# HybridRobotics/ilqr-iterative-tasks

Hardware: AMD Instinct MI355X
Metric: batched iLQR iterations/s (n=6,m=2,N=20) (higher is better)
Workload: dtype f64

## Files before the change

### ilqr_iterative_tasks_amd/csrc/i2lqr_abi.hip

```cpp
#include <hip/hip_runtime.h>
#include <dlfcn.h>
#include <rccl/rccl.h>

#include <atomic>
#include <cmath>
#include <cstdarg>
#include <cstdio>
#include <cstdlib>
#include <cstring>
#include <mutex>
#include <new>
#include <unordered_set>

#include "../../include/i2lqr.h"
#include "i2lqr_devcfg.hpp"
#include "i2lqr_geometry.hpp"
#include "i2lqr_group.h"
#include "i2lqr_lane.hpp"
#include "i2lqr_select.hpp"
#include "i2lqr_wave.hpp"

#include "i2lqr_lane12.h"

#define I2LQR_DRY_RUN_LANE 1
// ... 173 lines not shown
int debug_check(int rc, void* stream) {
#ifdef I2LQR_DEBUG
  if (rc != I2LQR_OK) return rc;
  unsigned long long* w = i2lqr::debug_trap_word();
  if (!w) return rc;
  hipStreamCaptureStatus cap = hipStreamCaptureStatusNone;
  if (hipStreamIsCapturing((hipStream_t)stream, &cap) == hipSuccess &&
      cap != hipStreamCaptureStatusNone)
    return rc;
  if (hipStreamSynchronize((hipStream_t)stream) != hipSuccess)
    return fail(I2LQR_ERR_LAUNCH, "debug build: the stream reported an error");
  unsigned long long rec = 0;
  if (hipMemcpy(&rec, w, sizeof(rec), hipMemcpyDeviceToHost) != hipSuccess)
    return fail(I2LQR_ERR_LAUNCH, "debug build: could not read the violation record");
  if (rec) {
    (void)hipMemset(w, 0, sizeof(rec));
    static const char* const names[] = {"?", "wave-kernel LDS slice", "eight-lane LDS slice",
                                        "sixteen-lane LDS slice", "quad12 HBM workspace slot",
                                        "lane kernel row of X", "lane kernel row of U / k",
                                        "lane kernel row of K", "lane kernel LDS word",
                                        "compaction row / problem index"};
    const int tag = (int)((rec >> 56) & 0x7f);
    return fail(I2LQR_ERR_LAUNCH, "debug build: index check failed: %s, index %lld, limit %lld",
                names[tag < 10 ? tag : 0], (long long)((rec >> 28) & 0xfffffff),
                (long long)(rec & 0xfffffff));
  }
#else
  (void)stream;
#endif
  return rc;
}
}

struct i2lqr_handle {
  i2lqr_config cfg;
  int lanes;
  size_t lds_bytes;
  int device;
  void* ws;
  int64_t ws_bytes;
  int64_t compact_min_batch;
  int opt_defer, opt_reroll, opt_lds_steps, opt_merge, opt_ckpt, opt_stagger;
  int wave_tail;
  int opt_pair;
  int opt_two_x;
  int opt_chunk_step;
  int opt_fuse;
  int opt_final_round;
  int opt_first_chunk;
  int opt_fstep;
  int opt_group;
  int opt_spec;
  int opt_group_ws;
  struct Epilogue {
    const int32_t* qfun;
    int outer_iter, max_relax_iter;
    void* cost_it;
    void* part;
    int64_t* best_idx;
    void* best_cost;
    bool fused;
  };
  static constexpr unsigned kTickets = 16;
  unsigned* ticket;
  std::atomic<unsigned> ticket_next;
  hipEvent_t ev_ready, ev_side_done;
  bool side_pending;
  DeviceGeometry geo;
};

namespace {
thread_local i2lqr_handle::Epilogue* t_epi = nullptr;
}

namespace {

enum FusedKernel { K_WAVE, K_GROUP, K_GROUP16, K_GROUP_WS, K_SPEC, K_SPEC16, K_QUAD, K_INVALID };
constexpr int64_t kAutoGroupBatch = 1024;
constexpr int64_t kAutoSpecBatch = 12288;

FusedKernel select_fused(const i2lqr_handle* h, int64_t B, bool early_exit, const char** why) {
  static const char* none = "";
  if (!why) why = &none;
  const bool m2 = h->cfg.m == 2 && h->cfg.n + h->cfg.m <= 8;
  const bool q16 = h->cfg.n + h->cfg.m == 16;
  if (m2) {
    const bool can = group_supported(h->cfg);
    if (h->opt_group == 8 && !can) {
      *why = "\"group_lanes\" = 8 needs a bicycle plant with Q = R = 0 and a horizon whose eight "
             "problem slices fit a CU's LDS";
      return K_INVALID;
    }
    const bool can_spec16 = group_spec_supported(h->cfg, 16), can_spec8 = group_spec_supported(h->cfg, 8);
    const bool spec16 = h->opt_group == 16 || (h->opt_group < 0 && can_spec16);
    const bool can_spec = spec16 ? can_spec16 : can_spec8;
    if (h->opt_spec == 1 && !can_spec) {
      *why = "\"speculate\" = 1 needs the eight- / sixteen-lane kernel and a horizon whose speculative "
             "buffers fit a CU's LDS";
      return K_INVALID;
    }
    if (can_spec && h->opt_group != 64 &&
        (h->opt_spec == 1 ||
         (h->opt_spec < 0 && h->opt_group < 0 && early_exit && B <= h->geo.scaled(kAutoSpecBatch))))
      return spec16 ? K_SPEC16 : K_SPEC;
    const bool can16 = group16_supported(h->cfg);
    if (h->opt_group == 16 && !can16) {
// ... 84 lines not shown
    IterArgs<T> a;
    a.B = B;
    a.n_iters = n_iters;
    a.early_exit = early_exit;
    a.X = (T*)X;
    a.U = (T*)U;
    a.x_term = (const T*)x_term;
    a.lamb = (T*)lamb;
    a.obs = (const T*)obs;
    a.cost = (T*)cost;
    a.K = (T*)K;
    a.k = (T*)k;
    a.iters = iters;
    a.status = status;
    a.dbg = nullptr;
    a.count = nullptr; a.count_max = 0; a.max_total = 0; a.set_stride = 0;
#ifdef I2LQR_STAMPS
    a.dbg = (unsigned long long*)h->ws;
#endif
    const char* why = "";
    const FusedKernel fk = select_fused(h, B, early_exit != 0, &why);
    if (t_epi && (fk == K_GROUP || fk == K_GROUP16 || fk == K_GROUP_WS)) {
      a.qfun = t_epi->qfun;
      a.outer_iter = t_epi->outer_iter;
      a.max_relax_iter = t_epi->max_relax_iter;
      a.cost_it = (T*)t_epi->cost_it;
      if (t_epi->best_idx) {
        a.pick_part = (MinPair<T>*)t_epi->part;
        a.pick_ticket = h->ticket + h->ticket_next.fetch_add(1, std::memory_order_relaxed) %
                                        i2lqr_handle::kTickets;
        a.best_idx = t_epi->best_idx;
        a.best_cost = (T*)t_epi->best_cost;
      }
      t_epi->fused = true;
    }
    switch (fk) {
      case K_INVALID:
        return fail(I2LQR_ERR_UNSUPPORTED, "%s", why);
      case K_SPEC:
      case K_SPEC16:
        if constexpr (m == 2 && n + m <= 8) {
          HIP_TRY(group_spec_iterate<T>(h->cfg, a, s, fk == K_SPEC16 ? 16 : 8));
          return I2LQR_OK;
        }
        break;
      case K_GROUP:
        if constexpr (m == 2 && n + m <= 8) {
          HIP_TRY(group_iterate<T>(h->cfg, a, s));
          return I2LQR_OK;
        }
        break;
      case K_GROUP16:
        if constexpr (m == 2 && n + m <= 8) {
          HIP_TRY(group16_iterate<T>(h->cfg, a, s));
          return I2LQR_OK;
        }
        break;
      case K_GROUP_WS:
        if constexpr (m == 2 && n + m <= 8) {
          HIP_TRY(group_iterate_ws<T>(h->cfg, a, h->ws, s));
          return I2LQR_OK;
        }
        break;
      case K_QUAD:
        if constexpr (n + m == 16) {
          HIP_TRY(quad_iterate<T>(h->cfg, a, h->ws, s));
          return I2LQR_OK;
        }
        break;
      case K_WAVE:
        break;
    }
    const size_t lds_f = fstep_lds_bytes(h->cfg.N);
    const int64_t waves_per_cu = (grid(B) + h->geo.cus - 1) / h->geo.cus;
    const bool fstep = kHasFstep && lds_f <= h->geo.default_dyn_lds &&
                       (h->opt_fstep >= 0 ? h->opt_fstep != 0
                                          : waves_per_cu * lds_f <= h->geo.lds_per_cu - 10 * 1024);
    if constexpr (kHasFstep) {
      if (fstep) {
        if (c.flags)
          hipLaunchKernelGGL((k_iterate<T, Sys, LANES, true, true>), dim3(grid(B)), dim3(64), lds_f,
                             s, c, a);
        else
          hipLaunchKernelGGL((k_iterate<T, Sys, LANES, false, true>), dim3(grid(B)), dim3(64), lds_f,
                             s, c, a);
        HIP_TRY(hipGetLastError());
        return I2LQR_OK;
      }
    }
    if (c.flags)
      hipLaunchKernelGGL((k_iterate<T, Sys, LANES, true>), dim3(grid(B)), dim3(64), h->lds_bytes, s,
                         c, a);
    else
      hipLaunchKernelGGL((k_iterate<T, Sys, LANES, false>), dim3(grid(B)), dim3(64), h->lds_bytes,
                         s, c, a);
    HIP_TRY(hipGetLastError());
    return I2LQR_OK;
  }
  static int names_pair(i2lqr_handle*, int64_t, int) { return 0; }
  static int solve_chained(i2lqr_handle* h, int64_t L, int k, void* X, void* U, const void* x_term,
                           void* lamb, const void* obs, void* cost, void* K, void* kk, int32_t* iters,
                           int32_t* status, hipStream_t s) {
    if constexpr (m == 2 && n + m <= 8) {
      if (h->opt_spec == 0 || h->opt_group == 8 || h->opt_group == 64 ||
          !group_spec_chain_supported(h->cfg, L))
        return fail(I2LQR_ERR_UNSUPPORTED, "chains run on the sixteen-lane speculative kernel: a "
                    "bicycle plant with Q = R = 0, at most %lld chains, a horizon whose three-wavefront "
// ... 879 lines not shown
    case I2LQR_SYS_QUAD12: n = 12; m = 4; break;
    default: return fail(I2LQR_ERR_INVALID, "unknown system_id %d", cfg->system_id);
  }
  if (cfg->n != n || cfg->m != m)
    return fail(I2LQR_ERR_INVALID, "system %d has n=%d m=%d, config says n=%d m=%d", cfg->system_id,
                n, m, cfg->n, cfg->m);
  if (cfg->N < 1 || cfg->N > I2LQR_MAX_HORIZON)
    return fail(I2LQR_ERR_INVALID, "horizon %d outside [1, %d]", cfg->N, I2LQR_MAX_HORIZON);
  if (cfg->dtype != I2LQR_F64 && cfg->dtype != I2LQR_F32)
    return fail(I2LQR_ERR_INVALID, "unknown dtype %d", cfg->dtype);
  if (cfg->layout != I2LQR_LAYOUT_PROBLEM_MAJOR && cfg->layout != I2LQR_LAYOUT_BATCH_MINOR &&
      cfg->layout != I2LQR_LAYOUT_BATCH_TILED)
    return fail(I2LQR_ERR_INVALID, "unknown layout %d", cfg->layout);
  if (!(cfg->dt > 0) || !(cfg->lamb_factor > 1) || cfg->max_iter < 0)
    return fail(I2LQR_ERR_INVALID, "need dt > 0, lamb_factor > 1, max_iter >= 0");
  for (int a = 0; a < m; a++)
    if (!(cfg->u_max[a] > 0)) return fail(I2LQR_ERR_INVALID, "u_max[%d] must be > 0", a);
  if (cfg->layout != I2LQR_LAYOUT_PROBLEM_MAJOR) {
    for (int i = 0; i < n; i++)
      for (int j = 0; j < i; j++)
        if (cfg->Q[i * I2LQR_MAX_N + j] != cfg->Q[j * I2LQR_MAX_N + i] ||
            cfg->Qt[i * I2LQR_MAX_N + j] != cfg->Qt[j * I2LQR_MAX_N + i])
          return fail(I2LQR_ERR_UNSUPPORTED, "the batch-minor / batch-tiled layouts need "
                      "symmetric Q and Qterminal (use the problem-major layout otherwise)");
    for (int a = 0; a < m; a++)
      for (int b = 0; b < a; b++)
        if (cfg->R[a * I2LQR_MAX_M + b] != cfg->R[b * I2LQR_MAX_M + a])
          return fail(I2LQR_ERR_UNSUPPORTED, "the batch-minor / batch-tiled layouts need a "
                      "symmetric R (use the problem-major layout otherwise)");
  }
  int ndev = 0;
#ifdef I2LQR_DRY_RUN
  const bool dry_run = dry::on();
#else
  constexpr bool dry_run = false;
#endif
  if (!dry_run && (hipGetDeviceCount(&ndev) != hipSuccess || ndev <= 0))
    return fail(I2LQR_ERR_NODEVICE, "no HIP device visible (this library has no CPU path)");
  i2lqr_handle* h = new (std::nothrow) i2lqr_handle;
  if (!h) return fail(I2LQR_ERR_LAUNCH, "out of host memory");
  h->cfg = *cfg;
  h->geo = device_geometry();
  if (h->geo.wave != 64) {
    const int w = h->geo.wave;
    delete h;
    return fail(I2LQR_ERR_UNSUPPORTED, "the kernels are built for 64-lane wavefronts (gfx950), this "
                "device reports %d", w);
  }
  h->ws = nullptr;
  h->ws_bytes = 0;
  h->compact_min_batch = -1;
  h->opt_defer = h->opt_reroll = h->opt_lds_steps = h->opt_fstep = h->opt_group = -1;
  h->opt_merge = h->opt_ckpt = h->opt_spec = h->opt_stagger = h->opt_group_ws = -1;
  h->wave_tail = -1;
  h->opt_first_chunk = -1;
  h->opt_fuse = -1;
  h->opt_final_round = -1;
  h->opt_chunk_step = -1;
  h->opt_pair = -1;
  h->opt_two_x = -1;
  h->ticket = nullptr;
  h->ticket_next.store(0);
  h->ev_ready = h->ev_side_done = nullptr;
  h->side_pending = false;
  constexpr size_t kTicketBytes = i2lqr_handle::kTickets * sizeof(unsigned);
  if (dry_run) {
#ifdef I2LQR_DRY_RUN
    static unsigned fake_tickets[i2lqr_handle::kTickets];
    h->device = 0;
    h->ticket = fake_tickets;
    dry::allow(fake_tickets, sizeof(fake_tickets));
#endif
  } else if (hipGetDevice(&h->device) != hipSuccess ||
      hipMalloc((void**)&h->ticket, kTicketBytes) != hipSuccess ||
      hipMemset(h->ticket, 0, kTicketBytes) != hipSuccess) {
    if (h->ticket) (void)hipFree(h->ticket);
    delete h;
    return fail(I2LQR_ERR_LAUNCH, "could not set up the handle's device state: %s",
                hipGetErrorString(hipGetLastError()));
  }
  const int rc = prepare_dispatch(h);
  if (rc != I2LQR_OK) {
    (void)hipFree(h->ticket);
    delete h;
    return rc;
  }
  {
    std::lock_guard<std::mutex> lock(g_live_mu);
    live_handles().insert(h);
  }
  *out = h;
  g_err[0] = 0;
  return I2LQR_OK;
}

int64_t i2lqr_dry_run(int32_t op, void* p, int64_t n) {
#ifdef I2LQR_DRY_RUN
  switch (op) {
    case 0: return dry::on() ? 1 : 0;
    case 1: if (!dry::on()) break; dry::allow(p, (size_t)n); return 0;
    case 2: if (!dry::on()) break; dry::reset(); return 0;
    case 3: if (!dry::on()) break; return dry::report((char*)p, n);
    default: return fail(I2LQR_ERR_INVALID, "i2lqr_dry_run: unknown operation %d", op);
  }
  return fail(I2LQR_ERR_UNSUPPORTED, "dry-run launches need I2LQR_DRY_RUN=1 in the environment");
#else
// ... 94 lines not shown
  for (int a = 0; a < cfg->m; a++)
    for (int b = 0; b < cfg->m; b++) {
      if (cfg->R[a * I2LQR_MAX_M + b] != 0.0) weights = true;
      if (cfg->R[a * I2LQR_MAX_M + b] != cfg->R[b * I2LQR_MAX_M + a]) lane_ok = false;
    }
  int64_t from;
  switch (cfg->system_id) {
    case I2LQR_SYS_BICYCLE4:
    case I2LQR_SYS_BICYCLE6:
      from = weights ? kLaneFromWeights
                     : (early_exit ? lane_from(*cfg).solve : lane_from(*cfg).iterate);
      break;
    case I2LQR_SYS_QUAD12: {
      const LaneFrom q = kLaneFromQuad[cfg->N <= 31 ? 0 : 1][cfg->dtype == I2LQR_F64 ? 0 : 1];
      from = weights ? kLaneFromWeights : (early_exit ? q.solve : q.iterate);
      if (cfg->dtype != I2LQR_F64 && weights) lane_ok = false;
      break;
    }
    default: return fail(I2LQR_ERR_INVALID, "unknown system_id %d", cfg->system_id);
  }
  from = device_geometry().scaled_from(from);
  if (!lane_ok || B < from) return I2LQR_LAYOUT_PROBLEM_MAJOR;
  return B % 64 == 0 ? I2LQR_LAYOUT_BATCH_TILED : I2LQR_LAYOUT_BATCH_MINOR;
}

int i2lqr_set_compaction(i2lqr_handle* h, int64_t min_batch) {
  if (!h) return fail(I2LQR_ERR_INVALID, "null handle");
  if (h->cfg.layout == I2LQR_LAYOUT_PROBLEM_MAJOR && min_batch > 0)
    return fail(I2LQR_ERR_UNSUPPORTED, "compaction applies to the batch-minor / batch-tiled layouts");
  h->compact_min_batch = min_batch < 0 ? -1 : min_batch;
  return I2LQR_OK;
}

int i2lqr_set_option(i2lqr_handle* h, const char* name, int64_t value) {
  if (!h || !name) return fail(I2LQR_ERR_INVALID, "null handle or option name");
  if (value < -1 || value > 0x7fffffff) return fail(I2LQR_ERR_INVALID, "option value out of range");
  const int v = (int)value;
  if (!strcmp(name, "defer_states")) h->opt_defer = v < 0 ? -1 : (v != 0);
  else if (!strcmp(name, "reroll_nominal")) h->opt_reroll = v < 0 ? -1 : (v != 0);
  else if (!strcmp(name, "lds_gain_steps")) h->opt_lds_steps = v;
  else if (!strcmp(name, "merge_inputs")) h->opt_merge = v < 0 ? -1 : (v != 0);
  else if (!strcmp(name, "checkpoint_states")) h->opt_ckpt = v < 0 ? -1 : (v != 0);
  else if (!strcmp(name, "stagger")) h->opt_stagger = v;
  else if (!strcmp(name, "per_step_jacobians")) h->opt_fstep = v < 0 ? -1 : (v != 0);
  else if (!strcmp(name, "wave_tail")) h->wave_tail = v < 0 ? -1 : (v > 65536 ? 65536 : v);
  else if (!strcmp(name, "first_chunk")) h->opt_first_chunk = v < 1 ? -1 : (v > 1024 ? 1024 : v);
  else if (!strcmp(name, "helper_wavefront")) h->opt_pair = v < 0 ? -1 : (v != 0);
  else if (!strcmp(name, "state_buffers")) h->opt_two_x = v < 0 ? -1 : (v != 0);
  else if (!strcmp(name, "chunk_step")) h->opt_chunk_step = v < 1 ? -1 : (v > 1024 ? 1024 : v);
  else if (!strcmp(name, "fused_compaction")) h->opt_fuse = v < 0 ? -1 : (v != 0);
  else if (!strcmp(name, "final_round")) h->opt_final_round = v < 0 ? -1 : (v > 20 ? 20 : v);
  else if (!strcmp(name, "speculate")) h->opt_spec = v < 0 ? -1 : (v != 0);
  else if (!strcmp(name, "group_workspace")) h->opt_group_ws = v < 0 ? -1 : (v != 0);
  else if (!strcmp(name, "debug_self_test")) {
#ifdef I2LQR_DEBUG
    unsigned long long* w = i2lqr::debug_trap_word();
    double* buf = nullptr;
    HIP_TRY(hipMalloc((void**)&buf, 8 * sizeof(double)));
    hipLaunchKernelGGL(k_debug_self_test, dim3(1), dim3(64), 0, (hipStream_t)0, buf, w);
    const int rc = debug_check(I2LQR_OK, nullptr);
    (void)hipFree(buf);
    return rc;
#else
    return fail(I2LQR_ERR_UNSUPPORTED, "\"debug_self_test\" exists in the index-checked debug build "
                "only (make -C ilqr_iterative_tasks_amd/csrc debug)");
#endif
  }
  else if (!strcmp(name, "group_lanes")) {
    if (v != -1 && v != 8 && v != 16 && v != 64)
      return fail(I2LQR_ERR_INVALID, "\"group_lanes\" is 8, 16, 64 or -1");
    h->opt_group = v;
  }
  else return fail(I2LQR_ERR_INVALID, "unknown option '%s'", name);
  return I2LQR_OK;
}

static const char* kernel_name(const i2lqr_handle* h, int64_t B, bool early_exit) {
  if (!h) return "";
  if (h->cfg.layout != I2LQR_LAYOUT_PROBLEM_MAJOR) {
    if (h->cfg.system_id == I2LQR_SYS_QUAD12) return "k_lane_iterate_rows";
    return names_pair_dispatch(const_cast<i2lqr_handle*>(h), B, early_exit ? 1 : 0) == 1
               ? "k_lane_iterate_pair" : "k_lane_iterate";
  }
  switch (select_fused(h, B, early_exit, nullptr)) {
    case K_SPEC: return "k_group_spec";
    case K_SPEC16: return "k_group_spec (sixteen lanes)";
    case K_GROUP: return "k_group_iterate";
    case K_GROUP16: return "k_group_iterate (sixteen lanes)";
    case K_GROUP_WS: return "k_group_iterate (workspace form)";
    case K_QUAD: return "k_quad_iterate";
    case K_WAVE: return "k_iterate";
    default: return "unsupported";
  }
}

const char* i2lqr_iterate_kernel(const i2lqr_handle* h, int64_t B) { return kernel_name(h, B, false); }
const char* i2lqr_solve_kernel(const i2lqr_handle* h, int64_t B) { return kernel_name(h, B, true); }

int i2lqr_set_workspace(i2lqr_handle* h, void* workspace, int64_t bytes) {
  if (!h) return fail(I2LQR_ERR_INVALID, "null handle");
  if (bytes < 0 || (bytes > 0 && !workspace) || ((uintptr_t)workspace & 15))
    return fail(I2LQR_ERR_INVALID, "workspace must be a 16-byte aligned device pointer");
  h->ws = workspace;
  h->ws_bytes = bytes;
  return I2LQR_OK;
}
// ... 545 lines not shown
```

### ilqr_iterative_tasks_amd/csrc/i2lqr_group.h

```cpp
#pragma once
#include <hip/hip_runtime.h>

#include "../../include/i2lqr.h"
#include "i2lqr_wave.hpp"

namespace i2lqr {

bool group_supported(const i2lqr_config& cfg);
template <class T> hipError_t group_iterate(const i2lqr_config& cfg, const IterArgs<T>& a,
                                            hipStream_t stream);

constexpr int64_t kGroup16Batch = 4096;
bool group16_supported(const i2lqr_config& cfg);
template <class T> hipError_t group16_iterate(const i2lqr_config& cfg, const IterArgs<T>& a,
                                              hipStream_t stream);

constexpr int64_t kGroupWsBatch = 4096;
constexpr int64_t kGroupWsTop = 8192;
constexpr int64_t kGroupWsTopF32 = 7168;
inline int64_t group_ws_top(const i2lqr_config& cfg) {
  return cfg.dtype == I2LQR_F64 ? kGroupWsTop : kGroupWsTopF32;
}
int64_t group_workspace_bytes(const i2lqr_config& cfg, int64_t B);
template <class T> hipError_t group_iterate_ws(const i2lqr_config& cfg, const IterArgs<T>& a,
                                               void* ws, hipStream_t stream);

bool group_spec_supported(const i2lqr_config& cfg, int lanes);
template <class T> hipError_t group_spec_iterate(const i2lqr_config& cfg, const IterArgs<T>& a,
                                                 hipStream_t stream, int lanes);
bool group_spec_chain_supported(const i2lqr_config& cfg, int64_t chains);
template <class T> hipError_t group_spec_chain(const i2lqr_config& cfg, const IterArgs<T>& a,
                                               hipStream_t stream);
bool group_spec_tail_supported(const i2lqr_config& cfg);
template <class T> hipError_t group_spec_tail(const i2lqr_config& cfg, const IterArgs<T>& a,
                                              hipStream_t stream);

bool quad_supported(const i2lqr_config& cfg);
int64_t quad_workspace_bytes(const i2lqr_config& cfg, int64_t B);
template <class T> hipError_t quad_iterate(const i2lqr_config& cfg, const IterArgs<T>& a, void* ws,
                                           hipStream_t stream);

}
```

### ilqr_iterative_tasks_amd/csrc/i2lqr_group.hip

```cpp
#include "i2lqr_group.h"

#include "i2lqr_devcfg.hpp"
#include "i2lqr_geometry.hpp"
#include "i2lqr_group.hpp"
#include "i2lqr_dryrun.hpp"

namespace i2lqr {

namespace {

template <class T, class Sys, int G = kGroup> size_t group_lds_bytes(int N) {
  return (size_t)GLayout<Sys, G>(N).wave_words() * sizeof(T);
}

bool has_stage_weights(const i2lqr_config& cfg) {
  for (int i = 0; i < cfg.n; i++)
    for (int j = 0; j < cfg.n; j++)
      if (cfg.Q[i * I2LQR_MAX_N + j] != 0.0) return true;
  for (int a = 0; a < cfg.m; a++)
    for (int b = 0; b < cfg.m; b++)
      if (cfg.R[a * I2LQR_MAX_M + b] != 0.0) return true;
  return false;
}

template <auto Kernel> hipError_t raise_lds_limit(size_t lds) {
  if (lds <= device_geometry().default_dyn_lds) return hipSuccess;
  constexpr int kMaxDev = 64;
  static thread_local int raised_for[kMaxDev] = {};
  int dev = 0;
  hipError_t e = hipGetDevice(&dev);
  if (e != hipSuccess) return e;
  if (dev < 0 || dev >= kMaxDev || raised_for[dev] < (int)lds) {
    e = hipFuncSetAttribute((const void*)Kernel, hipFuncAttributeMaxDynamicSharedMemorySize,
                            (int)lds);
    if (e != hipSuccess) return e;
    if (dev >= 0 && dev < kMaxDev) raised_for[dev] = (int)lds;
  }
  return hipSuccess;
}

template <class T, class Sys, int H, int G = kGroup>
hipError_t launch_h(const i2lqr_config& cfg, const IterArgs<T>& a, hipStream_t s) {
  const auto c = make_dev_cfg<T, Sys::n, Sys::m>(cfg);
  const size_t lds = group_lds_bytes<T, Sys, G>(cfg.N);
  if (hipError_t e = raise_lds_limit<k_group_iterate<T, Sys, H, false, G>>(lds); e != hipSuccess)
    return e;
  constexpr int PW = 64 / G;
  const unsigned grid = (unsigned)((a.B + PW - 1) / PW);
  hipLaunchKernelGGL((k_group_iterate<T, Sys, H, false, G>), dim3(grid), dim3(64 * H), lds, s, c, a,
                     (T*)nullptr);
  return hipGetLastError();
}
template <class T, class Sys>
hipError_t launch16(const i2lqr_config& cfg, const IterArgs<T>& a, hipStream_t s) {
  const int64_t cus = device_geometry().cus;
#ifndef I2LQR_STAMPS
  if ((a.B + 3) / 4 <= 2 * cus) return launch_h<T, Sys, 2, 16>(cfg, a, s);
#endif
  return launch_h<T, Sys, 1, 16>(cfg, a, s);
}
template <class T, class Sys>
hipError_t launch_ws(const i2lqr_config& cfg, const IterArgs<T>& a, void* ws, hipStream_t s) {
  const auto c = make_dev_cfg<T, Sys::n, Sys::m>(cfg);
  const size_t lds = (size_t)GLayout<Sys>(cfg.N, true).wave_words() * sizeof(T);
  if (hipError_t e = raise_lds_limit<k_group_iterate<T, Sys, 1, true>>(lds); e != hipSuccess) return e;
  const unsigned grid = (unsigned)((a.B + kGroupsPerWave - 1) / kGroupsPerWave);
  hipLaunchKernelGGL((k_group_iterate<T, Sys, 1, true>), dim3(grid), dim3(64), lds, s, c, a, (T*)ws);
  return hipGetLastError();
}

template <class T, class Sys>
hipError_t launch(const i2lqr_config& cfg, const IterArgs<T>& a, hipStream_t s) {
  const int64_t cus = device_geometry().cus;
#ifndef I2LQR_STAMPS
  if ((a.B + kGroupsPerWave - 1) / kGroupsPerWave <= cus) return launch_h<T, Sys, 3>(cfg, a, s);
#endif
  return launch_h<T, Sys, 1>(cfg, a, s);
}

constexpr int kSpecWideBatch = 512;

template <class T, class Sys, int V, int G = kGroup> size_t spec_lds_bytes(int N) {
  return (size_t)GSpecLayout<Sys, V, G>(N).group_words() * sizeof(T);
}

template <class T, class Sys, int V, bool SETIO, int G>
hipError_t launch_spec_v(const i2lqr_config& cfg, const IterArgs<T>& a, hipStream_t s) {
  const auto c = make_dev_cfg<T, Sys::n, Sys::m>(cfg);
  const size_t lds = spec_lds_bytes<T, Sys, V, G>(cfg.N);
  if (hipError_t e = raise_lds_limit<k_group_spec<T, Sys, V, SETIO, G>>(lds); e != hipSuccess)
    return e;
  constexpr int PW = 64 / G;
  const int64_t problems = SETIO ? (int64_t)a.count_max : a.B;
  const unsigned grid = (unsigned)((problems + PW - 1) / PW);
  hipLaunchKernelGGL((k_group_spec<T, Sys, V, SETIO, G>), dim3(grid), dim3(64 * V), lds, s, c, a);
  return hipGetLastError();
}
template <class T, class Sys, bool SETIO, int G>
hipError_t launch_spec(const i2lqr_config& cfg, const IterArgs<T>& a, hipStream_t s) {
  const DeviceGeometry& geo = device_geometry();
  const bool wide = !SETIO && a.B <= geo.scaled(kSpecWideBatch) &&
                    spec_lds_bytes<T, Sys, 3, G>(cfg.N) <= geo.max_dyn_lds;
  if (wide) return launch_spec_v<T, Sys, 3, SETIO, G>(cfg, a, s);
  return launch_spec_v<T, Sys, 2, SETIO, G>(cfg, a, s);
}
template <class T, bool SETIO>
hipError_t launch_spec_any(const i2lqr_config& cfg, const IterArgs<T>& a, hipStream_t s, int lanes) {
  const bool b4 = cfg.system_id == I2LQR_SYS_BICYCLE4;
  if (lanes == 16)
// ... 38 lines not shown
  hipLaunchKernelGGL((k_group_spec<T, Sys, 3, false, 16, true>), dim3(grid), dim3(64 * 3), lds, s, c, a);
  return hipGetLastError();
}
bool group_spec_chain_supported(const i2lqr_config& cfg, int64_t chains) {
  if (!spec_plant_ok(cfg) || cfg.layout != I2LQR_LAYOUT_PROBLEM_MAJOR) return false;
  const DeviceGeometry& geo = device_geometry();
  if (chains > geo.scaled(kSpecWideBatch)) return false;
  const size_t lds = cfg.dtype == I2LQR_F64
      ? (cfg.system_id == I2LQR_SYS_BICYCLE4 ? spec_lds_bytes<double, Bicycle4<double>, 3, 16>(cfg.N)
                                             : spec_lds_bytes<double, Bicycle6<double>, 3, 16>(cfg.N))
      : (cfg.system_id == I2LQR_SYS_BICYCLE4 ? spec_lds_bytes<float, Bicycle4<float>, 3, 16>(cfg.N)
                                             : spec_lds_bytes<float, Bicycle6<float>, 3, 16>(cfg.N));
  return lds <= geo.max_dyn_lds;
}
template <> hipError_t group_spec_chain<double>(const i2lqr_config& cfg, const IterArgs<double>& a,
                                                hipStream_t s) {
  if (cfg.system_id == I2LQR_SYS_BICYCLE4) return launch_spec_chain<double, Bicycle4<double>>(cfg, a, s);
  return launch_spec_chain<double, Bicycle6<double>>(cfg, a, s);
}
template <> hipError_t group_spec_chain<float>(const i2lqr_config& cfg, const IterArgs<float>& a,
                                               hipStream_t s) {
  if (cfg.system_id == I2LQR_SYS_BICYCLE4) return launch_spec_chain<float, Bicycle4<float>>(cfg, a, s);
  return launch_spec_chain<float, Bicycle6<float>>(cfg, a, s);
}

template <> hipError_t group_spec_iterate<double>(const i2lqr_config& cfg, const IterArgs<double>& a,
                                                  hipStream_t s, int lanes) {
  return launch_spec_any<double, false>(cfg, a, s, lanes);
}
template <> hipError_t group_spec_iterate<float>(const i2lqr_config& cfg, const IterArgs<float>& a,
                                                 hipStream_t s, int lanes) {
  return launch_spec_any<float, false>(cfg, a, s, lanes);
}
template <> hipError_t group_spec_tail<double>(const i2lqr_config& cfg, const IterArgs<double>& a,
                                               hipStream_t s) {
  return launch_spec_any<double, true>(cfg, a, s, group_spec_tail_lanes(cfg));
}
template <> hipError_t group_spec_tail<float>(const i2lqr_config& cfg, const IterArgs<float>& a,
                                              hipStream_t s) {
  return launch_spec_any<float, true>(cfg, a, s, group_spec_tail_lanes(cfg));
}

bool group16_supported(const i2lqr_config& cfg) {
  if (cfg.system_id != I2LQR_SYS_BICYCLE4 && cfg.system_id != I2LQR_SYS_BICYCLE6) return false;
  if (cfg.layout != I2LQR_LAYOUT_PROBLEM_MAJOR || has_stage_weights(cfg)) return false;
  const size_t lds = cfg.dtype == I2LQR_F64
      ? (cfg.system_id == I2LQR_SYS_BICYCLE4 ? group_lds_bytes<double, Bicycle4<double>, 16>(cfg.N)
                                             : group_lds_bytes<double, Bicycle6<double>, 16>(cfg.N))
      : (cfg.system_id == I2LQR_SYS_BICYCLE4 ? group_lds_bytes<float, Bicycle4<float>, 16>(cfg.N)
                                             : group_lds_bytes<float, Bicycle6<float>, 16>(cfg.N));
  return lds <= device_geometry().max_dyn_lds;
}
template <> hipError_t group16_iterate<double>(const i2lqr_config& cfg, const IterArgs<double>& a,
                                               hipStream_t s) {
  if (cfg.system_id == I2LQR_SYS_BICYCLE4) return launch16<double, Bicycle4<double>>(cfg, a, s);
  return launch16<double, Bicycle6<double>>(cfg, a, s);
}
template <> hipError_t group16_iterate<float>(const i2lqr_config& cfg, const IterArgs<float>& a,
                                              hipStream_t s) {
  if (cfg.system_id == I2LQR_SYS_BICYCLE4) return launch16<float, Bicycle4<float>>(cfg, a, s);
  return launch16<float, Bicycle6<float>>(cfg, a, s);
}

bool group_supported(const i2lqr_config& cfg) {
  if (cfg.system_id != I2LQR_SYS_BICYCLE4 && cfg.system_id != I2LQR_SYS_BICYCLE6) return false;
  if (cfg.layout != I2LQR_LAYOUT_PROBLEM_MAJOR || has_stage_weights(cfg)) return false;
  const size_t lds = cfg.dtype == I2LQR_F64
      ? (cfg.system_id == I2LQR_SYS_BICYCLE4 ? group_lds_bytes<double, Bicycle4<double>>(cfg.N)
                                             : group_lds_bytes<double, Bicycle6<double>>(cfg.N))
      : (cfg.system_id == I2LQR_SYS_BICYCLE4 ? group_lds_bytes<float, Bicycle4<float>>(cfg.N)
                                             : group_lds_bytes<float, Bicycle6<float>>(cfg.N));
  return lds <= device_geometry().max_dyn_lds;
}

int64_t group_workspace_bytes(const i2lqr_config& cfg, int64_t B) {
  if (!group_supported(cfg) || B <= 0) return 0;
  const int64_t probs = (B + kGroupsPerWave - 1) / kGroupsPerWave * kGroupsPerWave;
  const int64_t words = cfg.system_id == I2LQR_SYS_BICYCLE4
      ? GLayout<Bicycle4<double>>(cfg.N, true).ws_words()
      : GLayout<Bicycle6<double>>(cfg.N, true).ws_words();
  const size_t lds = cfg.dtype == I2LQR_F64
      ? (cfg.system_id == I2LQR_SYS_BICYCLE4
             ? (size_t)GLayout<Bicycle4<double>>(cfg.N, true).wave_words() * 8
             : (size_t)GLayout<Bicycle6<double>>(cfg.N, true).wave_words() * 8)
      : (cfg.system_id == I2LQR_SYS_BICYCLE4
             ? (size_t)GLayout<Bicycle4<float>>(cfg.N, true).wave_words() * 4
             : (size_t)GLayout<Bicycle6<float>>(cfg.N, true).wave_words() * 4);
  if (lds > device_geometry().max_dyn_lds) return 0;
  return probs * words * (cfg.dtype == I2LQR_F64 ? 8 : 4);
}
template <> hipError_t group_iterate_ws<double>(const i2lqr_config& cfg, const IterArgs<double>& a,
                                                void* ws, hipStream_t s) {
  if (cfg.system_id == I2LQR_SYS_BICYCLE4) return launch_ws<double, Bicycle4<double>>(cfg, a, ws, s);
  return launch_ws<double, Bicycle6<double>>(cfg, a, ws, s);
}
template <> hipError_t group_iterate_ws<float>(const i2lqr_config& cfg, const IterArgs<float>& a,
                                               void* ws, hipStream_t s) {
  if (cfg.system_id == I2LQR_SYS_BICYCLE4) return launch_ws<float, Bicycle4<float>>(cfg, a, ws, s);
  return launch_ws<float, Bicycle6<float>>(cfg, a, ws, s);
}

template <> hipError_t group_iterate<double>(const i2lqr_config& cfg, const IterArgs<double>& a,
                                             hipStream_t s) {
  if (cfg.system_id == I2LQR_SYS_BICYCLE4) return launch<double, Bicycle4<double>>(cfg, a, s);
  return launch<double, Bicycle6<double>>(cfg, a, s);
}
template <> hipError_t group_iterate<float>(const i2lqr_config& cfg, const IterArgs<float>& a,
                                            hipStream_t s) {
  if (cfg.system_id == I2LQR_SYS_BICYCLE4) return launch<float, Bicycle4<float>>(cfg, a, s);
  return launch<float, Bicycle6<float>>(cfg, a, s);
}

}
```

### ilqr_iterative_tasks_amd/csrc/i2lqr_group.hpp

```cpp
#pragma once
#include <hip/hip_runtime.h>
#include <stdint.h>

#include "i2lqr_systems.hpp"
#include "i2lqr_wave.hpp"

namespace i2lqr {

constexpr int kGroup = 8;
constexpr int kGroupsPerWave = 64 / kGroup;

template <class Sys> struct GroupPattern {
  static constexpr int n = Sys::n, m = Sys::m, W = n + m, NV = Sys::NVAR;
  static constexpr int dt_row(int b) {
    for (int i = 2; i < n; i++)
      if (i != b && Sys::pat(i, b) == 2) return i;
    return -1;
  }
  static constexpr bool column_ok(int b) {
    int extra = 0;
    for (int i = 0; i < n; i++) {
      const int code = Sys::pat(i, b);
      if (i < 2) {
        if (code == 2) return false;
// ... 419 lines not shown
          Kt[a * GL::KW + gcol] = kc[a];
          if (commit) Kg[a * GL::KW + gcol] = kc[a];
        }
      } else {
#pragma unroll
        for (int a = 0; a < m; a++)
          if (commit) Kt[a * GL::KW + gcol] = kc[a];
      }
      wave_sync();
      STAMP_END(4);
      T kr[m][n];
#pragma unroll
      for (int a = 0; a < m; a++)
#pragma unroll
        for (int i = 0; i < n; i++) kr[a][i] = Kt[a * GL::KW + i];
      if constexpr (!WS) load_record(t > 0 ? t - 1 : 0, rn);
      T qk[m];
#pragma unroll
      for (int a = 0; a < m; a++) {
        T acc = T(0);
#pragma unroll
        for (int b = 0; b < m; b++) acc = t_fma(Quu[a * m + b], kc[b], acc);
        qk[a] = acc;
      }
#pragma unroll
      for (int i = 0; i < n; i++) {
        T acc = T(0);
#pragma unroll
        for (int a = 0; a < m; a++) acc = t_fma(kr[a][i], qk[a], acc);
        va[i] = h[i] - acc;
      }
      STAMP_END(5);
    };
    int t = N - 1;
    if constexpr (I2LQR_GROUP_UNROLL >= 4) {
      for (; t >= 3; t -= 4) {
        step(t, ra, rb);
        step(t - 1, rb, ra);
        step(t - 2, ra, rb);
        step(t - 3, rb, ra);
      }
    }
    for (; t >= 1; t -= 2) {
      step(t, ra, rb);
      step(t - 1, rb, ra);
    }
    if (t == 0) step(0, ra, rb);
    ws_publish();
    return bad;
  }

  template <bool GENERAL>
  __device__ __forceinline__ bool backward_row(int XUo, const T (&xT)[n], T lamb, bool commit) const {
    static_assert(GL::KW > n + 1, "the padding word of a gain row takes the stores of idle lanes");
    bool bad = false;
    T va[n];
    {
      const T* Rn = rec(N);
      T dx[n];
#pragma unroll
      for (int i = 0; i < n; i++) dx[i] = S[XUo + N * W + i] - xT[i];
      const int gq = g < n ? g : 0;
#pragma unroll
      for (int i = 0; i < n; i++) {
        T vx = T(0);
#pragma unroll
        for (int r = 0; r < n; r++) vx += (T(2) * Qt[i * n + r]) * dx[r];
        const T vxx = T(2) * Qt[i * n + gq];
        va[i] = (g == n) ? vx : (g < n ? vxx : T(0));
      }
      va[0] += Rn[off_l0];
      va[1] += Rn[off_l1];
    }
    const int gcol = (commit && g <= n) ? g : GL::KW - 1;
    T cdr[n];
#pragma unroll
    for (int r = 0; r < n; r++) cdr[r] = (rsrc == r) ? cdt : T(0);
    struct Rec { T jv[NV], luu[m], c0, c1, l0, l1, lrow[m]; };
    Rec ra, rb;
    auto load_record = [&](int t, Rec& r) __attribute__((always_inline)) {
      const T* R = rec(t);
#pragma unroll
      for (int q = 0; q < NV; q++) r.jv[q] = R[GL::R_JV + q];
#pragma unroll
      for (int a = 0; a < m; a++) r.luu[a] = R[GL::R_LUU + a];
      r.c0 = R[off_c0];
      r.c1 = R[off_c1];
      r.l0 = R[off_l0];
      r.l1 = R[off_l1];
#pragma unroll
      for (int a = 0; a < m; a++) r.lrow[a] = R[off_lu[a]];
    };
    auto f_entry = [&](auto k_, auto b_, const T (&jv)[NV]) __attribute__((always_inline)) {
      constexpr int code = Sys::pat(decltype(k_)::value, n + decltype(b_)::value);
      if constexpr (code == 1) return T(1);
      else if constexpr (code == 2) return c.dt;
      else return jv[code >= 3 ? code - 3 : 0];
    };
    load_record(N - 1, ra);
    auto step = [&](const int t, Rec& rc, Rec& rn) __attribute__((always_inline)) {
      const T (&jv)[NV] = rc.jv;
      T t1[W];
      static_for_i<0, W>([&](auto a_) {
        constexpr int a = decltype(a_)::value;
        T acc = T(0);
        bool first = true;
        static_for_i<0, n>([&](auto i_) {
          constexpr int i = decltype(i_)::value;
          f_acc<i, a>(acc, first, va[i], jv);
        });
        t1[a] = acc;
      });
      dpp_ready(t1);
      load_record(t > 0 ? t - 1 : 0, rn);
      T Quu[m * m], Qinv[m * m];
      {
        T t1u[m];
#pragma unroll
        for (int a = 0; a < m; a++) t1u[a] = t1[n + a];
        static_for_i<0, m>([&](auto b_) {
          constexpr int b = decltype(b_)::value;
          T col[m];
#pragma unroll
// ... 208 lines not shown
      Sys::template trig_g<GENERAL>(x, tr, bad);
#pragma unroll
      for (int q = 0; q < NT; q++) S[TRn + t * NT + q] = tr[q];
      Sys::step_tr(c, x, u, tr, xn);
#pragma unroll
      for (int i = 0; i < n; i++) S[XUn + (t + 1) * W + i] = xn[i];
#pragma unroll
      for (int i = 0; i < n; i++) x[i] = xn[i];
    };
    int t = 0;
    if constexpr (WS) {
      for (; t + 1 < N; t += 2) {
        step(t, ga, gb);
        step(t + 1, gb, ga);
      }
      if (t < N) step(t, ga, gb);
    } else {
      if constexpr (I2LQR_GROUP_UNROLL >= 4) {
        for (; t + 3 < N; t += 4) {
          step(t, ga, ga);
          step(t + 1, ga, ga);
          step(t + 2, ga, ga);
          step(t + 3, ga, ga);
        }
      }
      for (; t + 1 < N; t += 2) {
        step(t, ga, ga);
        step(t + 1, ga, ga);
      }
      if (t < N) step(t, ga, ga);
    }
    Sys::template trig_g<GENERAL>(x, tr, bad);
#pragma unroll
    for (int q = 0; q < NT; q++) S[TRn + N * NT + q] = tr[q];
    const T cost = terminal_cost(x, xT);
    wave_sync();
    return cost;
  }
};

__device__ __forceinline__ int idx_div(int e, int d, float rcp_d) {
  int q = (int)((float)e * rcp_d);
  const int r = e - q * d;
  q += (r >= d) ? 1 : 0;
  q -= (r < 0) ? 1 : 0;
  return q;
}

template <class T, class Sys, int H = 1, bool WS = false, int G = kGroup>
__global__ __launch_bounds__(64 * H) void k_group_iterate(const DevCfg<T, Sys::n, Sys::m> c,
                                                          const IterArgs<T> a, T* ws = nullptr) {
  static_assert(!(WS && H > 1), "the workspace form runs without helper wavefronts");
  constexpr int n = Sys::n, m = Sys::m, W = n + m;
  using GL = GLayout<Sys, G>;
  extern __shared__ __align__(16) unsigned char gsmem_raw[];
  T* smem = reinterpret_cast<T*>(gsmem_raw);
  const int lane = threadIdx.x & 63, hv = threadIdx.x >> 6;
#ifdef I2LQR_STAMPS
  unsigned long long st_k0, st_k1, st_k2, st_k3;
  asm volatile("s_memtime %0\n\ts_waitcnt lgkmcnt(0)" : "=s"(st_k0)::"memory");
#endif
  const int64_t prob0 = (int64_t)blockIdx.x * GL::PW + lane / G;
  const bool real = prob0 < a.B;
  const int64_t prob = real ? prob0 : a.B - 1;
  GroupWorker<T, Sys, WS, G> w(c, smem, lane);
  const int N = c.N, g = w.g;
  const float rN = 1.0f / (float)N, rN1 = 1.0f / (float)(N + 1), rnN = 1.0f / (float)(n * N);
  const GL& L = w.L;
  const auto S = w.S;
  if constexpr (WS) w.Wp = ws + prob0 * (int64_t)L.ws_words();

  if (H == 1 || hv == 0) {
    const T* gX = a.X + prob * (int64_t)(n * (N + 1));
    if (g < n) S[L.XU0 + g] = gX[g * (N + 1)];
    const T* gU = a.U + prob * (int64_t)(m * N);
    for (int e = g; e < m * N; e += G) {
      const int aa = idx_div(e, N, rN), t = e - aa * N;
      S[L.XU0 + t * W + n + aa] = gU[e];
    }
    for (int e = lane; e < n * n; e += 64) smem[L.qt_base() + e] = c.Qt[e];
  }
  T xT[n], ob[6];
#pragma unroll
  for (int i = 0; i < n; i++) xT[i] = a.x_term[prob * n + i];
#pragma unroll
  for (int q = 0; q < 6; q++) ob[q] = a.obs ? a.obs[prob * 6 + q] : T(q == 5 ? -1 : 1);
  T lamb = a.lamb[prob];
  wave_sync();

  int cur = 0;
  const T ob_pa = T(1) / (ob[2] * ob[2]), ob_pb = T(1) / (ob[3] * ob[3]);
  int* const ctl = reinterpret_cast<int*>(smem + L.ctl_base());
  if constexpr (H > 1) {
    if (hv > 0) {
      for (;;) {
        __syncthreads();
        const int flags = ctl[8];
        if (!(flags & 1)) break;
        if (flags & 2) {
          const int pc = ctl[lane / G];
          w.prep(pc ? L.XU1 : L.XU0, pc ? L.TR1 : L.TR0, ob, ob_pa, ob_pb, hv * G + g,
                 H * G);
        }
        __syncthreads();
      }
      return;
    }
  }
  T cost = w.rollout(L.XU0, L.TR0, xT);
  int it = 0, status = a.early_exit ? 2  : 0 ;
  T cost_ret = cost;
  bool fresh = true, active = a.n_iters > 0;
#ifdef I2LQR_STAMPS
  asm volatile("s_memtime %0\n\ts_waitcnt lgkmcnt(0)" : "=s"(st_k1)::"memory");
#endif
  while (__any(active)) {
    const int XUo = cur ? L.XU1 : L.XU0, XUn = cur ? L.XU0 : L.XU1;
    const int TRo = cur ? L.TR1 : L.TR0, TRn = cur ? L.TR0 : L.TR1;
#ifdef I2LQR_STAMPS
    {
      auto& st_t0 = w.st_t0; auto& st_t1 = w.st_t1; auto& st_acc = w.st_acc;
      STAMP_BEGIN();
      if (__any(fresh)) w.prep(XUo, TRo, ob, ob_pa, ob_pb, g, G);
      STAMP_END(0);
    }
#else
    if constexpr (H > 1) {
      const bool do_prep = __any(fresh);
      if (g == 0) ctl[lane / G] = cur;
      if (lane == 0) ctl[8] = 1 | (do_prep ? 2 : 0);
      __syncthreads();
      if (do_prep) w.prep(XUo, TRo, ob, ob_pa, ob_pb, g, H * G);
      __syncthreads();
    } else {
      if (__any(fresh)) w.prep(XUo, TRo, ob, ob_pa, ob_pb, g, G);
    }
#endif
    if (__builtin_expect(__any(w.template backward<false>(XUo, xT, lamb, active)), 0))
      w.template backward<true>(XUo, xT, lamb, active);
    T cost_new;
    {
#ifdef I2LQR_STAMPS
      auto& st_t0 = w.st_t0; auto& st_t1 = w.st_t1; auto& st_acc = w.st_acc;
      STAMP_BEGIN();
#endif
      bool big = false;
      cost_new = w.template forward<false>(XUo, XUn, TRn, xT, &big);
      if (__builtin_expect(__any(big), 0)) cost_new = w.template forward<true>(XUo, XUn, TRn, xT, &big);
#ifdef I2LQR_STAMPS
      STAMP_END(6);
#endif
    }
    {
      const bool acc = active && cost_new < cost, rej = active && !(cost_new < cost);
      const T lamb_dn = lamb / c.lamb_factor, lamb_up = lamb * c.lamb_factor;
      const bool conv = t_abs((cost_new - cost) / cost) < c.eps;
      it += active ? 1 : 0;
      fresh = acc;
      cur ^= acc ? 1 : 0;
      lamb = acc ? lamb_dn : (rej ? lamb_up : lamb);
      cost_ret = acc ? cost_new : (rej ? cost : cost_ret);
      cost = acc ? cost_new : cost;
      const bool stop_conv = acc && conv, stop_lamb = rej && lamb > c.max_lamb;
      const int ended = stop_conv ? 1 : 3;
      if (a.early_exit) {
        status = (stop_conv || stop_lamb) ? ended : status;
        active = active && !(stop_conv || stop_lamb);
      } else {
        status = (status == 0 && (stop_conv || stop_lamb)) ? ended : status;
      }
      active = active && it < a.n_iters;
    }
  }
#ifdef I2LQR_STAMPS
  asm volatile("s_memtime %0\n\ts_waitcnt lgkmcnt(0)" : "=s"(st_k2)::"memory");
#endif
  if constexpr (H > 1) {
    if (lane == 0) ctl[8] = 0;
    __syncthreads();
  }
  if (!t_isfinite(cost_ret)) status = 4;

  if (real) {
    const int XUo = cur ? L.XU1 : L.XU0;
    T* gX = a.X + prob * (int64_t)(n * (N + 1));
    for (int e = g; e < n * (N + 1); e += G) {
      const int i = idx_div(e, N + 1, rN1), t = e - i * (N + 1);
      gX[e] = S[XUo + t * W + i];
    }
    T* gU = a.U + prob * (int64_t)(m * N);
    for (int e = g; e < m * N; e += G) {
      const int aa = idx_div(e, N, rN), t = e - aa * N;
      gU[e] = S[XUo + t * W + n + aa];
    }
    if (a.K) {
      T* gK = a.K + prob * (int64_t)(m * n * N);
      for (int e = g; e < m * n * N; e += G) {
        const int aa = idx_div(e, n * N, rnN), r = e - aa * (n * N);
        const int j = idx_div(r, N, rN), t = r - j * N;
        gK[e] = w.gain(t)[aa * GL::KW + j];
      }
      T* gk = a.k + prob * (int64_t)(m * N);
      for (int e = g; e < m * N; e += G) {
        const int aa = idx_div(e, N, rN), t = e - aa * N;
        gk[e] = w.gain(t)[aa * GL::KW + n];
      }
    }
    if (g == 0) {
      a.lamb[prob] = lamb;
      a.cost[prob] = cost_ret;
      if (a.iters) a.iters[prob] = it;
      if (a.status) a.status[prob] = status;
    }
#ifdef I2LQR_STAMPS
    asm volatile("s_waitcnt vmcnt(0)\n\ts_memtime %0\n\ts_waitcnt lgkmcnt(0)" : "=s"(st_k3)::"memory");
    w.st_acc[2] = st_k1 - st_k0;
    w.st_acc[3] = st_k2 - st_k1;
    w.st_acc[4] = st_k3 - st_k2;
    if (a.dbg && g == 0)
      for (int q = 0; q < 8; q++) a.dbg[prob * 8 + q] = w.st_acc[q];
#endif
  }
  if (a.qfun) {
    const bool cand = real && g == 0;
    T ci = T(0);
    if (cand) {
      const int XUo = cur ? L.XU1 : L.XU0;
      double ss = 0.0;
#pragma unroll
      for (int i = 0; i < n; i++) {
        const double d = (double)S[XUo + N * W + i] - (double)xT[i];
        ss += d * d;
      }
      ci = (T)relax_cost_value(ss, a.qfun[prob], N, a.outer_iter, a.max_relax_iter);
      a.cost_it[prob] = ci;
    }
// ... 241 lines not shown
```

Measured before the change: 70.78 million.

## Add third helper wavefront to group16 kernel to overlap prep and gain writeback

For small batches (one block per CU), the 16-lane group kernel now launches with three wavefronts. The main wavefront computes only the terminal value base itself, and the other two split the prep work. After the solve loop those two helpers write the K/k gains to global memory, while the main wave stores X/U with a per-timestep layout. The aim is to take prep and epilogue stores off the main wavefront's critical path, at the cost of more LDS-synchronised wavefronts per block and a new code path.

```diff
diff --git a/ilqr_iterative_tasks_amd/csrc/i2lqr_abi.hip b/ilqr_iterative_tasks_amd/csrc/i2lqr_abi.hip
--- a/ilqr_iterative_tasks_amd/csrc/i2lqr_abi.hip
+++ b/ilqr_iterative_tasks_amd/csrc/i2lqr_abi.hip
@@ -249,6 +249,7 @@
   int opt_group;
   int opt_spec;
   int opt_group_ws;
+  int opt_group_overlap;
   struct Epilogue {
     const int32_t* qfun;
     int outer_iter, max_relax_iter;
@@ -439,7 +440,7 @@
         break;
       case K_GROUP16:
         if constexpr (m == 2 && n + m <= 8) {
-          HIP_TRY(group16_iterate<T>(h->cfg, a, s));
+          HIP_TRY(group16_iterate<T>(h->cfg, a, s, h->opt_group_overlap != 0));
           return I2LQR_OK;
         }
         break;
@@ -1425,6 +1426,7 @@
   h->compact_min_batch = -1;
   h->opt_defer = h->opt_reroll = h->opt_lds_steps = h->opt_fstep = h->opt_group = -1;
   h->opt_merge = h->opt_ckpt = h->opt_spec = h->opt_stagger = h->opt_group_ws = -1;
+  h->opt_group_overlap = -1;
   h->wave_tail = -1;
   h->opt_first_chunk = -1;
   h->opt_fuse = -1;
@@ -1625,6 +1627,7 @@
   else if (!strcmp(name, "final_round")) h->opt_final_round = v < 0 ? -1 : (v > 20 ? 20 : v);
   else if (!strcmp(name, "speculate")) h->opt_spec = v < 0 ? -1 : (v != 0);
   else if (!strcmp(name, "group_workspace")) h->opt_group_ws = v < 0 ? -1 : (v != 0);
+  else if (!strcmp(name, "group_overlap")) h->opt_group_overlap = v < 0 ? -1 : (v != 0);
   else if (!strcmp(name, "debug_self_test")) {
 #ifdef I2LQR_DEBUG
     unsigned long long* w = i2lqr::debug_trap_word();
diff --git a/ilqr_iterative_tasks_amd/csrc/i2lqr_group.h b/ilqr_iterative_tasks_amd/csrc/i2lqr_group.h
--- a/ilqr_iterative_tasks_amd/csrc/i2lqr_group.h
+++ b/ilqr_iterative_tasks_amd/csrc/i2lqr_group.h
@@ -13,7 +13,7 @@
 constexpr int64_t kGroup16Batch = 4096;
 bool group16_supported(const i2lqr_config& cfg);
 template <class T> hipError_t group16_iterate(const i2lqr_config& cfg, const IterArgs<T>& a,
-                                              hipStream_t stream);
+                                              hipStream_t stream, bool overlap = true);
 
 constexpr int64_t kGroupWsBatch = 4096;
 constexpr int64_t kGroupWsTop = 8192;
diff --git a/ilqr_iterative_tasks_amd/csrc/i2lqr_group.hip b/ilqr_iterative_tasks_amd/csrc/i2lqr_group.hip
--- a/ilqr_iterative_tasks_amd/csrc/i2lqr_group.hip
+++ b/ilqr_iterative_tasks_amd/csrc/i2lqr_group.hip
@@ -52,9 +52,10 @@
   return hipGetLastError();
 }
 template <class T, class Sys>
-hipError_t launch16(const i2lqr_config& cfg, const IterArgs<T>& a, hipStream_t s) {
+hipError_t launch16(const i2lqr_config& cfg, const IterArgs<T>& a, hipStream_t s, bool overlap) {
   const int64_t cus = device_geometry().cus;
 #ifndef I2LQR_STAMPS
+  if (overlap && (a.B + 3) / 4 <= cus) return launch_h<T, Sys, 3, 16>(cfg, a, s);
   if ((a.B + 3) / 4 <= 2 * cus) return launch_h<T, Sys, 2, 16>(cfg, a, s);
 #endif
   return launch_h<T, Sys, 1, 16>(cfg, a, s);
@@ -199,14 +200,14 @@
   return lds <= device_geometry().max_dyn_lds;
 }
 template <> hipError_t group16_iterate<double>(const i2lqr_config& cfg, const IterArgs<double>& a,
-                                               hipStream_t s) {
-  if (cfg.system_id == I2LQR_SYS_BICYCLE4) return launch16<double, Bicycle4<double>>(cfg, a, s);
-  return launch16<double, Bicycle6<double>>(cfg, a, s);
+                                               hipStream_t s, bool overlap) {
+  if (cfg.system_id == I2LQR_SYS_BICYCLE4) return launch16<double, Bicycle4<double>>(cfg, a, s, overlap);
+  return launch16<double, Bicycle6<double>>(cfg, a, s, overlap);
 }
 template <> hipError_t group16_iterate<float>(const i2lqr_config& cfg, const IterArgs<float>& a,
-                                              hipStream_t s) {
-  if (cfg.system_id == I2LQR_SYS_BICYCLE4) return launch16<float, Bicycle4<float>>(cfg, a, s);
-  return launch16<float, Bicycle6<float>>(cfg, a, s);
+                                              hipStream_t s, bool overlap) {
+  if (cfg.system_id == I2LQR_SYS_BICYCLE4) return launch16<float, Bicycle4<float>>(cfg, a, s, overlap);
+  return launch16<float, Bicycle6<float>>(cfg, a, s, overlap);
 }
 
 bool group_supported(const i2lqr_config& cfg) {
diff --git a/ilqr_iterative_tasks_amd/csrc/i2lqr_group.hpp b/ilqr_iterative_tasks_amd/csrc/i2lqr_group.hpp
--- a/ilqr_iterative_tasks_amd/csrc/i2lqr_group.hpp
+++ b/ilqr_iterative_tasks_amd/csrc/i2lqr_group.hpp
@@ -495,23 +495,33 @@
 
   template <bool GENERAL>
   __device__ __forceinline__ bool backward_row(int XUo, const T (&xT)[n], T lamb, bool commit) const {
+    T vb[n];
+    terminal_base(XUo, xT, vb);
+    return backward_row_from<GENERAL>(vb, lamb, commit);
+  }
+  __device__ __forceinline__ void terminal_base(int XUo, const T (&xT)[n], T (&vb)[n]) const {
+    T dx[n];
+#pragma unroll
+    for (int i = 0; i < n; i++) dx[i] = S[XUo + N * W + i] - xT[i];
+    const int gq = g < n ? g : 0;
+#pragma unroll
+    for (int i = 0; i < n; i++) {
+      T vx = T(0);
+#pragma unroll
+      for (int r = 0; r < n; r++) vx += (T(2) * Qt[i * n + r]) * dx[r];
+      const T vxx = T(2) * Qt[i * n + gq];
+      vb[i] = (g == n) ? vx : (g < n ? vxx : T(0));
+    }
+  }
+  template <bool GENERAL>
+  __device__ __forceinline__ bool backward_row_from(const T (&vb)[n], T lamb, bool commit) const {
     static_assert(GL::KW > n + 1, "the padding word of a gain row takes the stores of idle lanes");
     bool bad = false;
     T va[n];
     {
       const T* Rn = rec(N);
-      T dx[n];
-#pragma unroll
-      for (int i = 0; i < n; i++) dx[i] = S[XUo + N * W + i] - xT[i];
-      const int gq = g < n ? g : 0;
-#pragma unroll
-      for (int i = 0; i < n; i++) {
-        T vx = T(0);
-#pragma unroll
-        for (int r = 0; r < n; r++) vx += (T(2) * Qt[i * n + r]) * dx[r];
-        const T vxx = T(2) * Qt[i * n + gq];
-        va[i] = (g == n) ? vx : (g < n ? vxx : T(0));
-      }
+#pragma unroll
+      for (int i = 0; i < n; i++) va[i] = vb[i];
       va[0] += Rn[off_l0];
       va[1] += Rn[off_l1];
     }
@@ -826,6 +836,11 @@
                                                           const IterArgs<T> a, T* ws = nullptr) {
   static_assert(!(WS && H > 1), "the workspace form runs without helper wavefronts");
   constexpr int n = Sys::n, m = Sys::m, W = n + m;
+#ifdef I2LQR_STAMPS
+  constexpr bool OVL = false;
+#else
+  constexpr bool OVL = G == 16 && H >= 3;
+#endif
   using GL = GLayout<Sys, G>;
   extern __shared__ __align__(16) unsigned char gsmem_raw[];
   T* smem = reinterpret_cast<T*>(gsmem_raw);
@@ -867,20 +882,43 @@
   int* const ctl = reinterpret_cast<int*>(smem + L.ctl_base());
   if constexpr (H > 1) {
     if (hv > 0) {
+      const int h0 = OVL ? hv - 1 : hv, hs = OVL ? H - 1 : H;
       for (;;) {
         __syncthreads();
         const int flags = ctl[8];
         if (!(flags & 1)) break;
         if (flags & 2) {
           const int pc = ctl[lane / G];
-          w.prep(pc ? L.XU1 : L.XU0, pc ? L.TR1 : L.TR0, ob, ob_pa, ob_pb, hv * G + g,
-                 H * G);
+          w.prep(pc ? L.XU1 : L.XU0, pc ? L.TR1 : L.TR0, ob, ob_pa, ob_pb, h0 * G + g, hs * G);
         }
         __syncthreads();
       }
+      if constexpr (OVL) {
+        if (real && a.K) {
+          T* const gK = a.K + prob * (int64_t)(m * n * N);
+          T* const gk = a.k + prob * (int64_t)(m * N);
+          for (int t = h0 * G + g; t < N; t += hs * G) {
+            const T* Kt = w.gain(t);
+            T kv[m][n + 1];
+#pragma unroll
+            for (int aa = 0; aa < m; aa++)
+#pragma unroll
+              for (int j = 0; j <= n; j++) kv[aa][j] = Kt[aa * GL::KW + j];
+#pragma unroll
+            for (int aa = 0; aa < m; aa++) {
+#pragma unroll
+              for (int j = 0; j < n; j++) gK[(aa * n + j) * N + t] = kv[aa][j];
+              gk[aa * N + t] = kv[aa][n];
+            }
+          }
+        }
+      }
       return;
     }
   }
+  T vb[n];
+#pragma unroll
+  for (int i = 0; i < n; i++) vb[i] = T(0);
   T cost = w.rollout(L.XU0, L.TR0, xT);
   int it = 0, status = a.early_exit ? 2  : 0 ;
   T cost_ret = cost;
@@ -904,14 +942,23 @@
       if (g == 0) ctl[lane / G] = cur;
       if (lane == 0) ctl[8] = 1 | (do_prep ? 2 : 0);
       __syncthreads();
-      if (do_prep) w.prep(XUo, TRo, ob, ob_pa, ob_pb, g, H * G);
+      if constexpr (OVL) {
+        if (do_prep) w.terminal_base(XUo, xT, vb);
+      } else {
+        if (do_prep) w.prep(XUo, TRo, ob, ob_pa, ob_pb, g, H * G);
+      }
       __syncthreads();
     } else {
       if (__any(fresh)) w.prep(XUo, TRo, ob, ob_pa, ob_pb, g, G);
     }
 #endif
-    if (__builtin_expect(__any(w.template backward<false>(XUo, xT, lamb, active)), 0))
-      w.template backward<true>(XUo, xT, lamb, active);
+    if constexpr (OVL) {
+      if (__builtin_expect(__any(w.template backward_row_from<false>(vb, lamb, active)), 0))
+        w.template backward_row_from<true>(vb, lamb, active);
+    } else {
+      if (__builtin_expect(__any(w.template backward<false>(XUo, xT, lamb, active)), 0))
+        w.template backward<true>(XUo, xT, lamb, active);
+    }
     T cost_new;
     {
 #ifdef I2LQR_STAMPS
@@ -955,7 +1002,29 @@
   }
   if (!t_isfinite(cost_ret)) status = 4;
 
-  if (real) {
+  if (OVL && real) {
+    const int XUo = cur ? L.XU1 : L.XU0;
+    T* const gX = a.X + prob * (int64_t)(n * (N + 1));
+    T* const gU = a.U + prob * (int64_t)(m * N);
+    for (int t = g; t <= N; t += G) {
+      T xu[W];
+#pragma unroll
+      for (int i = 0; i < W; i++) xu[i] = S[XUo + t * W + i];
+#pragma unroll
+      for (int i = 0; i < n; i++) gX[i * (N + 1) + t] = xu[i];
+      if (t < N) {
+#pragma unroll
+        for (int aa = 0; aa < m; aa++) gU[aa * N + t] = xu[n + aa];
+      }
+    }
+    if (g == 0) {
+      a.lamb[prob] = lamb;
+      a.cost[prob] = cost_ret;
+      if (a.iters) a.iters[prob] = it;
+      if (a.status) a.status[prob] = status;
+    }
+  }
+  if (!OVL && real) {
     const int XUo = cur ? L.XU1 : L.XU0;
     T* gX = a.X + prob * (int64_t)(n * (N + 1));
     for (int e = g; e < n * (N + 1); e += G) {
```

Result: faster. 74.78 million, median of 6 (+5.7%).
